# KIT-ISAS/lili-om

Measured on AMD Instinct MI355X. Metric: scan-to-map iterations/s (200k-pt scan vs 5M-pt map), higher is better.
Workload: dtype f64; 1 GPU; configs[2]: synthetic 64-ring 200000-pt scan vs 5000000-pt local map (variant A, seed 0x11110), ROT back-end matcher (surf), 1 outer GN iteration per step, a new registration from the perturbed pose every 10 steps, the 200k queries of the scan block-sharded over the ranks; queries_per_rank=200000, map_points=5000000, parallelism=single GPU, collectives=none, device_preheat_steps=2000

## Files before the change

lili_om_amd/csrc/lili_api.hip:

```cpp
#include "lili_launch.h"

#include <cmath>
#include <cstddef>
#include <cstdio>
#include <cstdlib>
#include <cstring>
#include <string>
#include <vector>

constexpr size_t kPinBytes = 64 * 1024;
namespace lili {
constexpr int kGatherMax = 12;
struct GatherTable { const unsigned char* src[kGatherMax]; unsigned off[kGatherMax], bytes[kGatherMax]; int n; };
__global__ __launch_bounds__(256) void k_readback_gather(GatherTable t, unsigned char* __restrict__ dst) {
    for (int k = 0; k < t.n; k++) {
        const unsigned char* s = t.src[k];
        unsigned char* d = dst + t.off[k];
        const unsigned nb = t.bytes[k];
        if (((reinterpret_cast<uintptr_t>(s) | reinterpret_cast<uintptr_t>(d) | nb) & 3u) == 0) {
            for (unsigned i = threadIdx.x; i < nb / 4; i += 256) reinterpret_cast<unsigned*>(d)[i] = reinterpret_cast<const unsigned*>(s)[i];
        } else for (unsigned i = threadIdx.x; i < nb; i += 256) d[i] = s[i];
    }
}
}
// ... 162 lines not shown
    if (!ctx) return LILI_E_ARG;
    HIPCHK(hipStreamSynchronize(ctx->stream));
    return LILI_OK;
}

int lili_set_debug(lili_ctx* ctx, int keep_neighbors) {
    if (!ctx) return LILI_E_ARG;
    ctx->keep_nn = keep_neighbors != 0;
    return LILI_OK;
}

int lili_set_option(lili_ctx* ctx, const char* name, int value) {
    if (!ctx || !name) return LILI_E_ARG;
    if (std::strcmp(name, "grid_reach") == 0) { if (value != 1 && value != 2) return ctx->fail(LILI_E_ARG, "grid_reach must be 1 or 2"); ctx->grid_reach = value; return LILI_OK; }
    if (std::strcmp(name, "cell_pct") == 0) { if (value < 50 || value > 100) return ctx->fail(LILI_E_ARG, "cell_pct must be in 50..100"); ctx->cell_pct = value; return LILI_OK; }
    if (std::strcmp(name, "fuse_tail") == 0) { ctx->fuse_tail = value != 0; return LILI_OK; }
    if (std::strcmp(name, "merge_kinds") == 0) { ctx->merge_kinds = value != 0; return LILI_OK; }
    if (std::strcmp(name, "fuse_lin") == 0) { ctx->fuse_lin = value != 0; return LILI_OK; }
    if (std::strcmp(name, "sort_fused_max_tiles") == 0) { ctx->sort_fused_max_tiles = std::max(0, value); return LILI_OK; }
    if (std::strcmp(name, "sort_fused_scan") == 0) { ctx->sort_fused_scan = value != 0; return LILI_OK; }
    if (std::strcmp(name, "persistent_iterate") == 0) { ctx->persistent_iterate = value != 0; return LILI_OK; }
    if (std::strcmp(name, "count_barrier") == 0) { ctx->count_barrier = value != 0; return LILI_OK; }
    if (std::strcmp(name, "assoc_lpq") == 0) {
        if (value != 0 && value != 1 && value != 2 && value != 4 && value != 8 && value != 16) return ctx->fail(LILI_E_ARG, "assoc_lpq must be 0 (auto), 1, 2, 4, 8 or 16");
        ctx->assoc_lpq = value; return LILI_OK;
    }
    if (std::strcmp(name, "fuse_lin_block") == 0) { if (value != 0 && value != kAssocBlock && value != kBlock) return ctx->fail(LILI_E_ARG, "fuse_lin_block must be 0 (auto), 64 or 256"); ctx->fuse_lin_block = value; return LILI_OK; }
    if (std::strcmp(name, "fine_grid") == 0) { ctx->fine_grid = value != 0; return LILI_OK; }
    if (std::strcmp(name, "sort_ride_hist") == 0) { ctx->sort_ride_hist = value != 0; return LILI_OK; }
    if (std::strcmp(name, "frame_guess_counts") == 0) { ctx->frame_guess_counts = value != 0; return LILI_OK; }
    if (std::strcmp(name, "frame_extract_stream") == 0) { ctx->frame_extract_stream = value != 0; return LILI_OK; }
    if (std::strcmp(name, "rot_fold") == 0) { ctx->rot_fold = value != 0; return LILI_OK; }
    if (std::strcmp(name, "rot_segment_wait") == 0) { ctx->rot_segment_wait = value != 0; return LILI_OK; }
    if (std::strcmp(name, "super_rows") == 0) { ctx->super_rows = value != 0; return LILI_OK; }
    if (std::strcmp(name, "fine_occupancy") == 0) { if (value < 2) return ctx->fail(LILI_E_ARG, "fine_occupancy must be >= 2"); ctx->fine_occupancy = value; return LILI_OK; }
    if (std::strcmp(name, "scan_lookback") == 0) { ctx->scan_lookback = value != 0; return LILI_OK; }
    if (std::strcmp(name, "map_narrow_counts") == 0) { ctx->map_narrow_counts = value != 0; for (auto& b : ctx->spec_box) b.wide_counts = false; return LILI_OK; }
    if (std::strcmp(name, "map_guess_box") == 0) { ctx->map_guess_box = value != 0; for (auto& b : ctx->spec_box) { const bool w = b.wide_counts; b = SpecBox{}; b.wide_counts = w; } return LILI_OK; }
    if (std::strcmp(name, "localmap_super_rows") == 0) { ctx->localmap_super_rows = value != 0; return LILI_OK; }
    if (std::strcmp(name, "localmap_incremental") == 0) { ctx->localmap_incremental = value != 0; return LILI_OK; }
    if (std::strcmp(name, "sort_digit_bits") == 0) { if (value != 4 && value != 8) return ctx->fail(LILI_E_ARG, "sort_digit_bits must be 4 or 8"); ctx->sort_digit_bits = value; return LILI_OK; }
    if (std::strcmp(name, "rot_atan") == 0) { if (value != 1 && value != 2) return ctx->fail(LILI_E_ARG, "rot_atan must be 1 or 2"); ctx->rot_atan = value; return LILI_OK; }
    if (std::strcmp(name, "p2p_fusion") == 0) { ctx->no_p2p_fusion = value == 0; return LILI_OK; }
    if (std::strcmp(name, "readback_gather") == 0) { ctx->readback_gather = value != 0; return LILI_OK; }
    if (std::strcmp(name, "voxel_guess_bits") == 0) { ctx->voxel_guess_bits = value != 0; return LILI_OK; }
    if (std::strcmp(name, "voxel_small") == 0) { ctx->voxel_small = value != 0; return LILI_OK; }
#ifdef LILI_OVERLAP_GN
    if (std::strcmp(name, "overlap_gn") == 0) { ctx->overlap_gn = value != 0; return LILI_OK; }
#endif
    if (std::strcmp(name, "archive_max_mb") == 0) { if (value < 0) return ctx->fail(LILI_E_ARG, "archive_max_mb must be >= 0 (0: unlimited)"); ctx->archive_max_mb = value; return LILI_OK; }
    if (std::strcmp(name, "archive_slab_mb") == 0) { if (value < 1 || value > 65536) return ctx->fail(LILI_E_ARG, "archive_slab_mb must be in 1..65536"); ctx->archive_slab_mb = value; return LILI_OK; }
    if (std::strcmp(name, "global_map_batch_points") == 0) {
        if (value < 1024 || value > (1 << 27)) return ctx->fail(LILI_E_ARG, "global_map_batch_points must be in 1024..2^27");
        ctx->global_map_batch_points = value; return LILI_OK;
    }
    if (std::strcmp(name, "max_cells") == 0) { if (value < 1) return ctx->fail(LILI_E_ARG, "max_cells must be positive"); ctx->max_cells = value; return LILI_OK; }
    return ctx->fail(LILI_E_ARG, std::string("unknown option ") + name);
}

}
```

lili_om_amd/csrc/lili_ctx.h:

```cpp
#pragma once
#include "../../include/lili_hip.h"
#include "lili_kernels.h"

#include <algorithm>
#include <cmath>
#include <cstdint>
#include <cstdlib>
#include <cstring>
#include <functional>
#include <string>
#include <utility>
#include <vector>

using namespace lili;

namespace lili_detail {

struct DevBuf {
    void* p = nullptr;
    size_t cap = 0;
    hipError_t ensure(size_t bytes) {
        if (bytes + 256 <= cap) return hipSuccess;
        if (p) { hipError_t e = hipFree(p); p = nullptr; cap = 0; if (e != hipSuccess) return e; }
        size_t want = bytes + bytes / 8 + 256;
// ... 112 lines not shown
    unsigned long long readback_gen = 0;
    struct PinItem { void* dst; size_t off, bytes; };
    std::vector<PinItem> h_pin_items;
    struct LazyItem { const void* src; size_t off, bytes; };
    std::vector<LazyItem> h_pin_lazy;
    unsigned char* h_pin_dev = nullptr;
    bool readback_gather = true;
    double* h_records = nullptr;
    double* h_records_dev = nullptr;
    int max_cells = 1 << 27;
    int grid_reach = 2;
    bool fuse_tail = false;
    bool no_p2p_fusion = false;
    bool merge_kinds = true;
    int cell_pct = 65;
    bool fine_grid = true;
    int fine_occupancy = 12;
    double focus[3] = {0, 0, 0}, focus_radius = 0;
    int fuse_lin_block = 0;
    int assoc_lpq = 0;
    bool count_barrier = false;

    bool persistent_off_now = false;
    bool persistent_iterate = false;
    bool frontend_commit_pending = false;
    int32_t frontend_map_raw = 0;
    bool voxel_guess_bits = true;
    bool hook_box_words_zero = false;
    std::function<int()> pre_sync_hook;
    bool voxel_small = true;
    bool overlap_gn = false;
    unsigned long long gn_seq = 0;
    bool fuse_lin = true;
    bool super_rows = true;
    bool scan_lookback = true;
    bool localmap_super_rows = false;
    bool localmap_incremental = true;
    int sort_fused_max_tiles = 256;
    bool sort_fused_scan = true;
    static constexpr int kExtractSide = 2;
    hipEvent_t extract_fork_ev = nullptr;
    bool frame_extract_stream = false, extract_side_next = false, extract_join_pending = false;
    bool rot_fold = true, rot_segment_wait = true;
    int frame_guess_misses = 0;
    bool frame_guess_counts = true;
    bool sort_ride_hist = true;
    int sort_digit_bits = 8;
    int rot_atan = 2;
    int n_simd = 0;
    void* ext_rot = nullptr;
    void (*ext_rot_free)(void*) = nullptr;
    void* ext_livox = nullptr;
    void (*ext_livox_free)(void*) = nullptr;
    void* ext_voxel = nullptr;
    void (*ext_voxel_free)(void*) = nullptr;
    void* ext_loop = nullptr;
    void (*ext_loop_free)(void*) = nullptr;
    void* ext_archive = nullptr;
    void (*ext_archive_free)(void*) = nullptr;
    int archive_max_mb = 0;
    int archive_slab_mb = 64;
    int global_map_batch_points = 1 << 21;

    int fail(int code, const std::string& m) { err = m; return code; }
    SlotState* state(int slot) { return states.as<SlotState>() + slot; }
    double* gram_of(int slot) { return gram.as<double>() + (size_t)slot * LILI_GRAM_DOUBLES; }
// ... 46 lines not shown
```

lili_om_amd/csrc/lili_kernels.h:

```cpp
#pragma once
#include <hip/hip_runtime.h>
#include <stdint.h>
#include "../../include/lili_hip.h"
#include "lili_p2p_dev.h"

namespace lili {

struct GridView {
    const float4* pts;
    const float* aux;
    const int* cell_start;
    const int* cell_start9;
    int bx0, by0, bz0, bnx, bny, bnz;
    double ox, oy, oz;
    double inv_cell;
    double cell;
    int nx, ny, nz;
    int n_points;
    int reach;
};

struct SrcCloud {
    const unsigned char* p;
    int stride, aux_off;
    int f4;
};

struct SlotState {
    double pose[7];
    int n_res[2];
    int gn_status;
    int iters;
    double last_delta[6];
    long long tprof[16];
    unsigned int reserved_;
    unsigned long long cnt_word;
    unsigned long long epoch;
    unsigned long long wait_failed;
};
constexpr int kPubReplicas = 64;
constexpr int kPubStride = 16;

struct FuseTail {
    int mode;
    const double* part_surf; int nb_surf;
    const double* part_edge; int nb_edge;
    double* out;
    SlotState* state;
    int debug;
    const SlotState* pose_src;
};

// ... 96 lines not shown
```

lili_om_amd/csrc/lili_match.hip:

```cpp
#include "lili_launch.h"

#include <cmath>
#include <cstddef>
#include <cstdio>
#include <cstdlib>
#include <cstring>
#include <string>
#include <type_traits>
#include <vector>

static MatchParams to_device_params(const lili_s2m_params* p) {
    MatchParams m{};
    m.variant = p->variant; m.loss = p->loss; m.loss_a = p->loss_a; m.lidar_const = p->lidar_const;
    m.kd_max_radius = p->kd_max_radius; m.edge_gate = p->edge_gate; m.surf_dist_thres = p->surf_dist_thres;
    m.reflect_thres = p->reflect_thres; m.surf_weight_min = p->surf_weight_min; m.edge_dist_max = p->edge_dist_max;
    for (int i = 0; i < 4; i++) m.q_lb[i] = p->q_lb[i];
    {
        const double w = p->q_lb[0], qx = p->q_lb[1], qy = p->q_lb[2], qz = p->q_lb[3];
        const double n2 = w * w + qx * qx + qy * qy + qz * qz;
        if (n2 > 0) { m.q_lb_inv[0] = w / n2; m.q_lb_inv[1] = -qx / n2; m.q_lb_inv[2] = -qy / n2; m.q_lb_inv[3] = -qz / n2; }
        else m.q_lb_inv[0] = m.q_lb_inv[1] = m.q_lb_inv[2] = m.q_lb_inv[3] = 0.0;
        const double gi = 1.0 / n2;
        if (n2 > 0) { m.q_lb_inv_jet[0] = w * gi; m.q_lb_inv_jet[1] = (-qx) * gi; m.q_lb_inv_jet[2] = (-qy) * gi; m.q_lb_inv_jet[3] = (-qz) * gi; }
        else m.q_lb_inv_jet[0] = m.q_lb_inv_jet[1] = m.q_lb_inv_jet[2] = m.q_lb_inv_jet[3] = 0.0;
// ... 28 lines not shown
    for (int i = 0; i < 4; i++) pa.q[i] = q[i];
    return pa;
}
static int derives_assoc(const lili_s2m_params* params) { return params->variant == LILI_VARIANT_FRONTEND ? 0 : 1; }
static PoseArg pose_of_slot(lili_ctx* ctx, int slot, const lili_s2m_params* assoc_params = nullptr, int pose_slot = -1) {
    PoseArg pa{};
    pa.state = ctx->state(pose_slot >= 0 ? pose_slot : slot);
    pa.derive_assoc = assoc_params ? derives_assoc(assoc_params) : 0;
    return pa;
}

static bool gate_fits(const MapIndex& m, int kind, const MatchParams& P) {
    const double gate = kind == LILI_KIND_SURF ? P.kd_max_radius : P.edge_gate;
    return std::sqrt(gate) * 1.0099 <= m.cell * (double)m.view.reach;
}
static bool livox_aux_ok(const MapIndex& m, const KindSlot& ks, int kind, const MatchParams& P) {
    return kind != LILI_KIND_SURF || P.variant != LILI_VARIANT_LIVOX || (m.has_aux && ks.has_aux);
}
static bool coop_eligible(lili_ctx* ctx, int slot, int kind_mask, const MatchParams& P, int64_t* n_all) {
    for (int kind = 0; kind < 2; kind++) if (kind_mask & (1 << kind)) {
        const KindSlot& ks = ctx->slots[slot].k[kind];
        const MapIndex& m = ctx->map[kind];
        if (!ks.has_queries || !m.valid || ks.n_q == 0 || m.n < 5 || m.has_fine) return false;
        if (!gate_fits(m, kind, P) || !livox_aux_ok(m, ks, kind, P)) return false;
        *n_all += ks.n_q;
    }
    return true;
}

static int assoc_args_of(lili_ctx* ctx, int slot, int kind, const GridView& view, int nb, int launches, AssocArgs& a) {
    KindSlot& ks = ctx->slots[slot].k[kind];
    const size_t n = (size_t)ks.n_q;
    a = AssocArgs{};
    a.queries = ks.q.as<float4>(); a.n_q = (int)n; a.g = view;
    a.rec0 = ks.rec0.as<float4>(); a.rec1 = ks.rec1.p; a.valid = ks.valid.as<unsigned char>();
    if (ctx->keep_nn) {
        HIPCHK(ks.dbg_idx.ensure(n * 5 * sizeof(int)));
        HIPCHK(ks.dbg_d2.ensure(n * 5 * sizeof(float)));
        a.dbg_idx = ks.dbg_idx.as<int>(); a.dbg_d2 = ks.dbg_d2.as<float>();
    }
    HIPCHK(ks.block_counts.ensure((size_t)nb * sizeof(int)));
    a.block_counts = ks.block_counts.as<int>(); a.nb = nb;
    ks.n_assoc_blocks = nb; ks.has_records = true; ks.launches += launches;
    return LILI_OK;
}
static int coop_args_of(lili_ctx* ctx, int slot, int kind_mask, int L, int launches, AssocArgs A[2]) {
    for (int kind = 0; kind < 2; kind++) {
        A[kind] = AssocArgs{};
        if (kind_mask & (1 << kind)) TRY(assoc_args_of(ctx, slot, kind, ctx->map[kind].view, nblocks(ctx->slots[slot].k[kind].n_q, 256 / L), launches, A[kind]));
    }
    return LILI_OK;
}

template <typename F> static bool with_lanes(int L, F&& f) {
    switch (L) {
        case 2: f(std::integral_constant<int, 2>{}); return true;
        case 4: f(std::integral_constant<int, 4>{}); return true;
        case 8: f(std::integral_constant<int, 8>{}); return true;
        case 16: f(std::integral_constant<int, 16>{}); return true;
        default: return false;
    }
}

constexpr size_t kHRecordDoubles = (size_t)LILI_MAX_SLOTS * LILI_GRAM_DOUBLES + 2 * LILI_MAX_SLOTS;
constexpr size_t kHWindowCountsOff = (size_t)LILI_MAX_SLOTS * LILI_GRAM_DOUBLES * sizeof(double), kHSlotCountsOff = kHWindowCountsOff + 2 * LILI_MAX_SLOTS * sizeof(int);
static int ensure_h_records(lili_ctx* ctx) {
    if (ctx->h_records) return LILI_OK;
// ... 1243 lines not shown
```

lili_om_amd/csrc/lili_s2m.hip:

```cpp
#include <type_traits>
#include "lili_kernels.h"
#include "lili_device_math.h"
#include "lili_device_cloud.h"
#include "lili_s2m_dev.h"

namespace lili {

__global__ __launch_bounds__(256) void k_cloud_to_f4(const unsigned char* __restrict__ raw, int n, int stride, int aux_off, float4* __restrict__ out, unsigned* __restrict__ mm) {
    float mn[3] = {INFINITY, INFINITY, INFINITY}, mx[3] = {-INFINITY, -INFINITY, -INFINITY};
    for (int i = blockIdx.x * blockDim.x + threadIdx.x; i < n; i += gridDim.x * blockDim.x) {
        const float4 v = load_row_f4(raw + (size_t)i * stride, aux_off);
        out[i] = v;
        if (mm && isfinite(v.x) && isfinite(v.y) && isfinite(v.z)) {
            mn[0] = fminf(mn[0], v.x); mn[1] = fminf(mn[1], v.y); mn[2] = fminf(mn[2], v.z);
            mx[0] = fmaxf(mx[0], v.x); mx[1] = fmaxf(mx[1], v.y); mx[2] = fmaxf(mx[2], v.z);
        }
    }
    if (!mm) return;
#pragma unroll
    for (int k = 0; k < 3; k++)
        for (int o = 32; o > 0; o >>= 1) { mn[k] = fminf(mn[k], __shfl_xor(mn[k], o)); mx[k] = fmaxf(mx[k], __shfl_xor(mx[k], o)); }
    __shared__ float smn[4][3], smx[4][3];
    if ((threadIdx.x & 63) == 0) {
#pragma unroll
// ... 546 lines not shown
        state->n_res[0] = t0; state->n_res[1] = t1;
        if (out) { out[0] = t0; out[1] = t1; }
    }
}



template <int BS, class TAB>
__device__ __forceinline__ void assoc_surf_body(
        const float4* __restrict__ queries, int n_q, const GridView& g, const PoseArg& pa, const MatchParams& P,
        float4* __restrict__ rec_nd, double* __restrict__ rec_score, unsigned char* __restrict__ valid,
        int* __restrict__ dbg_idx, float* __restrict__ dbg_d2, int* __restrict__ block_counts, int bid, TAB& tab, LaneRec* rec_out = nullptr) {
#ifdef LILI_PHASE_PROBE
    const long long t_begin = (P.debug & 4096) ? (long long)__builtin_amdgcn_s_memrealtime() : 0ll;
#endif
    const int i0 = bid * BS;
    const bool live = i0 + (int)threadIdx.x < n_q;
    const int i = live ? i0 + (int)threadIdx.x : 0;
    float4 ql = queries[i];
    dq Q2; d3 T2;
    load_assoc_pose(pa, P, Q2, T2);
    d3 pmd = qrot(Q2, d3{(double)ql.x, (double)ql.y, (double)ql.z}) + T2;
    float px = (float)pmd.x, py = (float)pmd.y, pz = (float)pmd.z;
    Top5 nn; nn.aux = 0; nn.have = false;
#ifdef LILI_PHASE_PROBE
    PhaseProbe probe;
#pragma unroll
    for (int k = 0; k < 8; k++) probe.t[k] = 0;
    PhaseProbe* const pp = &probe;
#else
    PhaseProbe* const pp = nullptr;
#endif
    PHASE_STAMP(pp, 1, px);
    if (live) knn5_grid(g, tab, px, py, pz, gate_bound(P.kd_max_radius), nn, P.debug, pp);
    bool ok = false;
    if (live) {
        store_debug_nn(g, nn, i, dbg_idx, dbg_d2);
        float4 rn; double score;
        ok = surf_fit(g, P, nn, ql, px, py, pz, rn, score);
        PHASE_STAMP(pp, 6, rn.w);
        rec_nd[i] = rn;
        rec_score[i] = score;
        valid[i] = ok ? 1 : 0;
        if (rec_out) { rec_out->ql = ql; rec_out->r0 = rn; rec_out->score = score; }
    }
    if (rec_out) rec_out->ok = ok;
    store_block_count<BS>(ok, block_counts, bid);
#ifdef LILI_PHASE_PROBE
    if ((P.debug & 4096) && dbg_d2 && threadIdx.x == 0) {
        for (int k = 1; k <= 6; k++) dbg_d2[(size_t)i0 * 5 + k] = probe.t[k] ? (float)(probe.t[k] - t_begin) : -1.0f;
    }
    if ((P.debug & 4096) && dbg_idx && threadIdx.x == 0) {
        long long* o = (long long*)(dbg_idx + (size_t)i0 * 5);
        unsigned hw, xcc;
        asm volatile("s_getreg_b32 %0, hwreg(HW_REG_HW_ID)" : "=s"(hw));
        asm volatile("s_getreg_b32 %0, hwreg(HW_REG_XCC_ID)" : "=s"(xcc));
        o[0] = t_begin; o[1] = (long long)__builtin_amdgcn_s_memrealtime();
        dbg_idx[(size_t)i0 * 5 + 4] = (int)((hw & 0xffffu) | (xcc << 16));
    }
    if ((P.debug & 4096) && dbg_idx && live && threadIdx.x != 0) dbg_idx[(size_t)i * 5] = nn.aux;
#endif
}
template <int BS>
__global__ __launch_bounds__(BS) void k_associate_surf(
        const float4* __restrict__ queries, int n_q, GridView g, PoseArg pa, MatchParams P,
        float4* __restrict__ rec_nd, double* __restrict__ rec_score, unsigned char* __restrict__ valid,
        int* __restrict__ dbg_idx, float* __restrict__ dbg_d2, int* __restrict__ block_counts) {
    __shared__ RowTabT<BS> tab;
    assoc_surf_body<BS>(queries, n_q, g, pa, P, rec_nd, rec_score, valid, dbg_idx, dbg_d2, block_counts, (int)blockIdx.x, tab);
}

template <int BS, class TAB>
__device__ __forceinline__ void assoc_edge_body(
        const float4* __restrict__ queries, int n_q, const GridView& g, const PoseArg& pa, const MatchParams& P,
        float4* __restrict__ rec_a, float4* __restrict__ rec_b, unsigned char* __restrict__ valid,
        int* __restrict__ dbg_idx, float* __restrict__ dbg_d2, int* __restrict__ block_counts, int bid, TAB& tab, LaneRec* rec_out = nullptr) {
    const int i0 = bid * BS;
    const bool live = i0 + (int)threadIdx.x < n_q;
    const int i = live ? i0 + (int)threadIdx.x : 0;
    float4 ql = queries[i];
    dq Q2; d3 T2;
    load_assoc_pose(pa, P, Q2, T2);
    d3 pmd = qrot(Q2, d3{(double)ql.x, (double)ql.y, (double)ql.z}) + T2;
    float px = (float)pmd.x, py = (float)pmd.y, pz = (float)pmd.z;
    Top5 nn; nn.have = false;
    if (live) knn5_grid(g, tab, px, py, pz, gate_bound(P.edge_gate), nn);
    bool ok = false;
    if (live) {
        store_debug_nn(g, nn, i, dbg_idx, dbg_d2);
        float4 ra, rb;
        ok = edge_fit(g, P, nn, px, py, pz, ra, rb);
        rec_a[i] = ra; rec_b[i] = rb; valid[i] = ok ? 1 : 0;
        if (rec_out) { rec_out->ql = ql; rec_out->r0 = ra; rec_out->r1 = rb; }
    }
    if (rec_out) rec_out->ok = ok;
    store_block_count<BS>(ok, block_counts, bid);
}
template <int BS>
__global__ __launch_bounds__(BS) void k_associate_edge(
        const float4* __restrict__ queries, int n_q, GridView g, PoseArg pa, MatchParams P,
        float4* __restrict__ rec_a, float4* __restrict__ rec_b, unsigned char* __restrict__ valid,
        int* __restrict__ dbg_idx, float* __restrict__ dbg_d2, int* __restrict__ block_counts) {
    __shared__ RowTabT<BS> tab;
    assoc_edge_body<BS>(queries, n_q, g, pa, P, rec_a, rec_b, valid, dbg_idx, dbg_d2, block_counts, (int)blockIdx.x, tab);
}

__global__ __launch_bounds__(kAssocBlock) void k_associate_both(AssocArgs S, AssocArgs E, PoseArg pa, MatchParams P) {
    __shared__ RowTabT<kAssocBlock> tab;
    const int b = (int)blockIdx.x;
    if (b < E.nb) assoc_edge_body<kAssocBlock>(E.queries, E.n_q, E.g, pa, P, E.rec0, reinterpret_cast<float4*>(E.rec1), E.valid, E.dbg_idx, E.dbg_d2, E.block_counts, b, tab);
    else assoc_surf_body<kAssocBlock>(S.queries, S.n_q, S.g, pa, P, S.rec0, reinterpret_cast<double*>(S.rec1), S.valid, S.dbg_idx, S.dbg_d2, S.block_counts, b - E.nb, tab);
}
template __global__ void k_associate_surf<kAssocBlock>(const float4*, int, GridView, PoseArg, MatchParams, float4*, double*, unsigned char*, int*, float*, int*);
template __global__ void k_associate_edge<kAssocBlock>(const float4*, int, GridView, PoseArg, MatchParams, float4*, float4*, unsigned char*, int*, float*, int*);


template <bool XCHG>
__device__ __forceinline__ void reduce_partials_block(const double* part_surf, int nb_surf, const double* part_edge, int nb_edge,
                                                      double* __restrict__ out, SlotState* __restrict__ state, int do_gn, unsigned long long key, const P2PView& xv,
// ... 463 lines not shown
```

lili_om_amd/csrc/lili_s2m_dev.h:

```cpp
#pragma once
#include <type_traits>
#include "lili_kernels.h"
#include "lili_device_math.h"

namespace lili {

__device__ __forceinline__ int cell_coord(float v, double o, double inv_cell) {
    return (int)floor(((double)v - o) * inv_cell);
}
__device__ __forceinline__ int cell_of(float4 p, const GridView& g) {
    if (!(isfinite(p.x) && isfinite(p.y) && isfinite(p.z))) return 0;
    int cx = min(max(cell_coord(p.x, g.ox, g.inv_cell), 0), g.nx - 1);
    int cy = min(max(cell_coord(p.y, g.oy, g.inv_cell), 0), g.ny - 1);
    int cz = min(max(cell_coord(p.z, g.oz, g.inv_cell), 0), g.nz - 1);
    return (cz * g.ny + cy) * g.nx + cx;
}

__device__ __forceinline__ size_t srow_index(const GridView& g, int x, int y, int z) {
    return ((size_t)(z - g.bz0) * (size_t)g.bny + (size_t)(y - g.by0)) * (size_t)g.bnx + (size_t)(x - g.bx0);
}

struct Top5 {
    float d[5];
    int j[5];
    int aux;
    float4 p[5];
    bool have;
};
__device__ __forceinline__ float dist2(float4 p, float qx, float qy, float qz) {
    float r = 0.f;
    float dx = qx - p.x; r += dx * dx;
    float dy = qy - p.y; r += dy * dy;
    float dz = qz - p.z; r += dz * dz;
    return r;
}
struct Sel5 {
    unsigned long long k[5];
    int j[5];
    __device__ __forceinline__ void init(float bound = 3.0e38f) {
        bound = fminf(bound, 3.0e38f);
#pragma unroll
        for (int s = 0; s < 5; s++) { k[s] = ((unsigned long long)__float_as_uint(bound) << 32) | 0x7fffffffull; j[s] = -1; }
    }
    __device__ __forceinline__ void insert(float d, float4 p, int jpos) {
        const unsigned long long key = ((unsigned long long)__float_as_uint(d) << 32) | (unsigned)__float_as_int(p.w);
        const bool c0 = key < k[0], c1 = key < k[1], c2 = key < k[2], c3 = key < k[3], c4 = key < k[4];
        k[4] = c3 ? k[3] : (c4 ? key : k[4]);  j[4] = c3 ? j[3] : (c4 ? jpos : j[4]);
        k[3] = c2 ? k[2] : (c3 ? key : k[3]);  j[3] = c2 ? j[2] : (c3 ? jpos : j[3]);
        k[2] = c1 ? k[1] : (c2 ? key : k[2]);  j[2] = c1 ? j[1] : (c2 ? jpos : j[2]);
        k[1] = c0 ? k[0] : (c1 ? key : k[1]);  j[1] = c0 ? j[0] : (c1 ? jpos : j[1]);
        k[0] = c0 ? key : k[0];                j[0] = c0 ? jpos : j[0];
    }
    __device__ __forceinline__ float worst() const { return __uint_as_float((unsigned)(k[4] >> 32)); }
    __device__ __forceinline__ bool final_tie() const { return false; }
    __device__ __forceinline__ unsigned worst_bits() const { return (unsigned)(k[4] >> 32); }
    __device__ __forceinline__ void to_top5(Top5& t) const {
#pragma unroll
        for (int s = 0; s < 5; s++) { t.d[s] = __uint_as_float((unsigned)(k[s] >> 32)); t.j[s] = j[s]; }
        t.have = false;
    }
};

__device__ __forceinline__ unsigned umed3(unsigned a, unsigned b, unsigned c) {
    unsigned r;
    asm("v_med3_u32 %0, %1, %2, %3" : "=v"(r) : "v"(a), "v"(b), "v"(c));
    return r;
}
struct Sel5K {
    unsigned k[6];
    int tc;
    int* T;
    int ts;
    unsigned bb;
    float bnd;
    __device__ __forceinline__ void init(float bound) {
        bnd = fminf(bound, 3.0e38f);
        bb = __float_as_uint(bnd) >> 6;
#pragma unroll
        for (int s = 0; s < 6; s++) k[s] = ((bb + 1u + (unsigned)s) << 6) | 63u;
        tc = 0; T = nullptr; ts = 0;
    }
    __device__ __forceinline__ void attach(int* col, int stride) { T = col; ts = stride; T[15 * stride] = -4; }
    __device__ __forceinline__ float worst() const { return __uint_as_float(k[4] | 63u); }
    __device__ __forceinline__ unsigned worst_bits() const { return k[4] | 63u; }
    __device__ __forceinline__ void to_top5(Top5& t) const {
#pragma unroll
        for (int s = 0; s < 5; s++) { t.d[s] = bnd; t.j[s] = -1; }
        t.have = false;
    }
    __device__ __forceinline__ void push(unsigned key) {
        const unsigned m5 = umed3(k[4], k[5], key), m4 = umed3(k[3], k[4], key), m3 = umed3(k[2], k[3], key);
        const unsigned m2 = umed3(k[1], k[2], key), m1 = umed3(k[0], k[1], key);
        k[0] = min(k[0], key); k[1] = m1; k[2] = m2; k[3] = m3; k[4] = m4; k[5] = m5;
    }
    __device__ __forceinline__ int where(unsigned key) const { const unsigned c = key & 63u; return T[(int)(c >> 2) * ts] + (int)(c & 3u); }
    __device__ __forceinline__ void repoint() {
        int jr[6];
#pragma unroll
        for (int s = 0; s < 6; s++) jr[s] = where(k[s]);
#pragma unroll
        for (int s = 0; s < 6; s++) { T[(8 + s) * ts] = jr[s]; k[s] = (k[s] & ~63u) | (unsigned)(32 + 4 * s); }
    }
    __device__ __forceinline__ void chunk(float4 p0, float4 p1, float4 p2, float4 p3, int j, int end, float qx, float qy, float qz) {
        if (tc >= 8 && (tc & 7) == 0) repoint();
        T[(tc & 7) * ts] = j;
        const unsigned code = (unsigned)(tc & 7) << 2;
        tc++;
        const unsigned u0 = __float_as_uint(dist2(p0, qx, qy, qz));
        const unsigned u1 = j + 1 < end ? __float_as_uint(dist2(p1, qx, qy, qz)) : 0x7f800000u;
        const unsigned u2 = j + 2 < end ? __float_as_uint(dist2(p2, qx, qy, qz)) : 0x7f800000u;
        const unsigned u3 = j + 3 < end ? __float_as_uint(dist2(p3, qx, qy, qz)) : 0x7f800000u;
        push((u0 & ~63u) | code); push((u1 & ~63u) | (code + 1u)); push((u2 & ~63u) | (code + 2u)); push((u3 & ~63u) | (code + 3u));
    }
    __device__ __forceinline__ bool finish(const GridView& g, float qx, float qy, float qz, Top5& t) const {
        const bool redo = ((k[5] ^ k[4]) < 64u) || ((k[4] >> 6) == bb);
        unsigned long long e[5];
        int jr[5];
        float4 pp[5];
#pragma unroll
        for (int s = 0; s < 5; s++) {
            jr[s] = where(k[s]);
            const bool real = jr[s] >= 0;
            const float4 p = g.pts[real ? jr[s] : 0];
            pp[s] = p;
            const unsigned du = real ? __float_as_uint(dist2(p, qx, qy, qz)) : __float_as_uint(bnd);
            const unsigned lo = real ? (unsigned)__float_as_int(p.w) : 0x7fffffffu;
            e[s] = ((unsigned long long)du << 32) | lo;
        }
        const bool unsorted = !(e[0] <= e[1] && e[1] <= e[2] && e[2] <= e[3] && e[3] <= e[4]);
        if (__any(unsorted)) {
#define LILI_CE(a, b) { const bool sw = e[b] < e[a]; const unsigned long long ea = e[a], eb = e[b]; const int ja = jr[a], jb = jr[b]; \
                        const float4 pa_ = pp[a], pb_ = pp[b]; \
                        e[a] = sw ? eb : ea; e[b] = sw ? ea : eb; jr[a] = sw ? jb : ja; jr[b] = sw ? ja : jb; \
                        pp[a].x = sw ? pb_.x : pa_.x; pp[a].y = sw ? pb_.y : pa_.y; pp[a].z = sw ? pb_.z : pa_.z; pp[a].w = sw ? pb_.w : pa_.w; \
                        pp[b].x = sw ? pa_.x : pb_.x; pp[b].y = sw ? pa_.y : pb_.y; pp[b].z = sw ? pa_.z : pb_.z; pp[b].w = sw ? pa_.w : pb_.w; }
            LILI_CE(0, 1) LILI_CE(3, 4) LILI_CE(2, 4) LILI_CE(2, 3) LILI_CE(0, 3) LILI_CE(0, 2) LILI_CE(1, 4) LILI_CE(1, 3) LILI_CE(1, 2)
#undef LILI_CE
        }
#pragma unroll
        for (int s = 0; s < 5; s++) { t.d[s] = __uint_as_float((unsigned)(e[s] >> 32)); t.j[s] = jr[s]; t.p[s] = pp[s]; }
        t.aux = tc;
        t.have = !redo;
        return redo;
    }
};
// ... 95 lines not shown
    if (u2 <= sel.worst_bits()) sel.insert(__uint_as_float(u2), p2, min(j + 2, last));
    if (u3 <= sel.worst_bits()) sel.insert(__uint_as_float(u3), p3, min(j + 3, last));
}
template <class SEL>
__device__ __forceinline__ void scan_run(const GridView& g, SEL& sel, int beg, int end, float qx, float qy, float qz) {
    const int last = end - 1;
    for (int j = beg; j < end; j += 4) {
        float4 p0 = load_pt(g, j), p1 = load_pt(g, min(j + 1, last)), p2 = load_pt(g, min(j + 2, last)), p3 = load_pt(g, min(j + 3, last));
        process_chunk(sel, p0, p1, p2, p3, j, end, qx, qy, qz);
    }
}

template <int BS>
struct RowTabT {
    int b[9][BS];
    int e[9][BS];
    float lb[9][BS];
    int cj[16][BS];
};

struct PhaseProbe { long long t[8]; };
#ifdef LILI_PHASE_PROBE
#define PHASE_STAMP(pp, k, dep) do { if (pp) { long long t_; asm volatile("s_memrealtime %0\n\ts_waitcnt lgkmcnt(0)" : "=s"(t_) : "v"(dep) : "memory"); (pp)->t[k] = t_; } } while (0)
#else
#define PHASE_STAMP(pp, k, dep) do {} while (0)
#endif
__device__ __forceinline__ float gate_bound(double gate) {
    float gf = (float)gate;
    if ((double)gf < gate) gf = __uint_as_float(__float_as_uint(gf) + 1u);
    return gf;
}
__device__ constexpr int kShellDy[16] = {0, 0, -2, 2, -1, 1, -1, 1, -2, -2, 2, 2, -2, -2, 2, 2};
__device__ constexpr int kShellDz[16] = {-2, 2, 0, 0, -2, -2, 2, 2, -1, 1, -1, 1, -2, 2, -2, 2};
template <class SEL, class TAB>
__device__ __forceinline__ bool knn5_grid_sel(const GridView& g, TAB& tab, float qx, float qy, float qz, float bound, Top5& best, PhaseProbe* pp = nullptr) {
    SEL sel; sel.init(bound);
    sel.to_top5(best);
    if (!(isfinite(qx) && isfinite(qy) && isfinite(qz))) return false;
    if constexpr (std::is_same<SEL, Sel5K>::value) sel.attach(&tab.cj[0][threadIdx.x], (int)(sizeof(tab.cj[0]) / sizeof(int)));
    const int R = g.reach;
    int cx = cell_coord(qx, g.ox, g.inv_cell), cy = cell_coord(qy, g.oy, g.inv_cell), cz = cell_coord(qz, g.oz, g.inv_cell);
    if (cx < -R || cx > g.nx - 1 + R || cy < -R || cy > g.ny - 1 + R || cz < -R || cz > g.nz - 1 + R) return false;
    const bool inner9 = g.cell_start9 && cy >= g.by0 && cy < g.by0 + g.bny && cz >= g.bz0 && cz < g.bz0 + g.bnz &&
                        max(cx - 1, 0) >= g.bx0 && min(cx + 1, g.nx - 1) < g.bx0 + g.bnx;
    if (inner9) {
        const int x0 = max(cx - 1, 0), x1 = min(cx + 1, g.nx - 1);
        if (x0 <= x1) {
            const int* row = g.cell_start9 + srow_index(g, g.bx0, cy, cz) - g.bx0;
            int cj = row[x0];
            const int ce = row[x1 + 1];
            PHASE_STAMP(pp, 2, ce);
            auto fetch = [&](float4& p0, float4& p1, float4& p2, float4& p3, int& pj) {
                pj = cj;
                const float4* q = (const float4*)((const char*)g.pts + ((unsigned)cj << 4));
                p0 = q[0]; p1 = q[1]; p2 = q[2]; p3 = q[3];
                cj += 4;
            };
            float4 a0, a1, a2, a3, b0, b1, b2, b3;
            int aj = 0, bj = 0;
            fetch(a0, a1, a2, a3, aj);
            for (;;) {
                if (!(aj < ce)) break;
                fetch(b0, b1, b2, b3, bj);
                process_chunk(sel, a0, a1, a2, a3, aj, ce, qx, qy, qz);
                if (!(bj < ce)) break;
                fetch(a0, a1, a2, a3, aj);
                process_chunk(sel, b0, b1, b2, b3, bj, ce, qx, qy, qz);
            }
        }
    } else {
        const int x0 = max(cx - 1, 0), x1 = min(cx + 1, g.nx - 1);
        if (x0 <= x1) {
            int rb[9], re[9];
#pragma unroll
            for (int n = 0; n < 9; n++) {
                const int w = row_order(n);
                const int y = cy + w / 3 - 1, z = cz + w % 3 - 1;
                const bool in = z >= 0 && z < g.nz && y >= 0 && y < g.ny;
// ... 18 lines not shown
                while (cj >= ce && n < cnt) {
                    const int b = tab.b[n][tid], e = tab.e[n][tid];
                    const float lb = tab.lb[n][tid];
                    n++;
                    if (!(lb > wv)) { cj = b; ce = e; }
                }
                pj = cj; pe = ce;
                if (cj < ce) {
                    const int last = ce - 1;
                    p0 = load_pt(g, cj); p1 = load_pt(g, min(cj + 1, last)); p2 = load_pt(g, min(cj + 2, last)); p3 = load_pt(g, min(cj + 3, last));
                    cj += 4;
                }
            };
            float4 a0, a1, a2, a3, b0, b1, b2, b3;
            int aj = 0, ae = 0, bj = 0, be = 0;
            fetch(sel.worst(), a0, a1, a2, a3, aj, ae);
            for (;;) {
                if (!(aj < ae)) break;
                fetch(sel.worst(), b0, b1, b2, b3, bj, be);
                process_chunk(sel, a0, a1, a2, a3, aj, ae, qx, qy, qz);
                if (!(bj < be)) break;
                fetch(sel.worst(), a0, a1, a2, a3, aj, ae);
                process_chunk(sel, b0, b1, b2, b3, bj, be, qx, qy, qz);
            }
        }
    }
    PHASE_STAMP(pp, 3, sel.worst());
    if (R == 2) {
        const double c = g.cell;
        const double fxm = (double)qx - (g.ox + (double)cx * c), fxp = (g.ox + (double)(cx + 1) * c) - (double)qx;
        const double fym = (double)qy - (g.oy + (double)cy * c), fyp = (g.oy + (double)(cy + 1) * c) - (double)qy;
        const double fzm = (double)qz - (g.oz + (double)cz * c), fzp = (g.oz + (double)(cz + 1) * c) - (double)qz;
        const double margin = c + fmax(fmin(fmin(fmin(fxm, fxp), fmin(fym, fyp)), fmin(fzm, fzp)), 0.0);
        if (!(sel.worst() < (float)(0.999 * margin * margin))) {
            const bool side9 = inner9 && (cx - 2 < 0 || cx - 2 >= g.bx0) && (cx + 2 >= g.nx || cx + 2 < g.bx0 + g.bnx);
            if (side9) {
                const int* row = g.cell_start9 + srow_index(g, g.bx0, cy, cz) - g.bx0;
                const int xl = cx - 2, xr = cx + 2;
                if (xl >= 0 && xl < g.nx) { const double gx = fmax(fxm + c, 0.0); if (!((float)(0.999 * gx * gx) > sel.worst())) scan_run(g, sel, row[xl], row[xl + 1], qx, qy, qz); }
                if (xr >= 0 && xr < g.nx) { const double gx = fmax(fxp + c, 0.0); if (!((float)(0.999 * gx * gx) > sel.worst())) scan_run(g, sel, row[xr], row[xr + 1], qx, qy, qz); }
            }
            const bool few = __popcll(__ballot(1)) <= 2;
            if (side9 && few) {
                const double g1m = fmax(fxm, 0.0), g1p = fmax(fxp, 0.0), g2m = fmax(fxm + c, 0.0), g2p = fmax(fxp + c, 0.0);
                const int tid = threadIdx.x;
#pragma unroll
                for (int batch = 0; batch < 2; batch++) {
                    const float wv = sel.worst();
                    int rb[8], re[8]; float rl[8];
#pragma unroll
                    for (int i = 0; i < 8; i++) {
                        const int dy = kShellDy[batch * 8 + i], dz = kShellDz[batch * 8 + i];
                        const int y = cy + dy, z = cz + dz;
                        const double gy = dy == 0 ? 0.0 : fmax(dy < 0 ? fym + (double)(-dy - 1) * c : fyp + (double)(dy - 1) * c, 0.0);
                        const double gz = dz == 0 ? 0.0 : fmax(dz < 0 ? fzm + (double)(-dz - 1) * c : fzp + (double)(dz - 1) * c, 0.0);
                        const double lbr = 0.999 * (gy * gy + gz * gz);
                        const int dl = (float)(lbr + 0.999 * g2m * g2m) > wv ? ((float)(lbr + 0.999 * g1m * g1m) > wv ? 0 : 1) : 2;
                        const int dr = (float)(lbr + 0.999 * g2p * g2p) > wv ? ((float)(lbr + 0.999 * g1p * g1p) > wv ? 0 : 1) : 2;
                        const int x0 = max(cx - dl, 0), x1 = min(cx + dr, g.nx - 1);
                        const bool keep = y >= 0 && y < g.ny && z >= 0 && z < g.nz && !((float)lbr > wv) && x0 <= x1;
                        const int* cs = g.cell_start + (size_t)(keep ? z * g.ny + y : 0) * g.nx;
                        const int b = cs[keep ? x0 : 0], e = cs[keep ? x1 + 1 : 0];
                        rb[i] = b; re[i] = keep ? e : b; rl[i] = (float)lbr;
                    }
#pragma unroll
                    for (int i = 0; i < 8; i++) { tab.b[i][tid] = rb[i]; tab.e[i][tid] = re[i]; tab.lb[i][tid] = rl[i]; }
                    for (int i = 0; i < 8; i++) {
                        const int b = tab.b[i][tid], e = tab.e[i][tid];
                        if (b < e && !(tab.lb[i][tid] > sel.worst())) scan_run(g, sel, b, e, qx, qy, qz);
                    }
                }
            } else
            for (int dz = -2; dz <= 2; dz++) {
                const int z = cz + dz;
                if (z < 0 || z >= g.nz) continue;
                const double gz = dz == 0 ? 0.0 : fmax(dz < 0 ? fzm + (double)(-dz - 1) * c : fzp + (double)(dz - 1) * c, 0.0);
                for (int dy = -2; dy <= 2; dy++) {
                    const int y = cy + dy;
                    if (y < 0 || y >= g.ny) continue;
                    const double gy = dy == 0 ? 0.0 : fmax(dy < 0 ? fym + (double)(-dy - 1) * c : fyp + (double)(dy - 1) * c, 0.0);
                    const double lbr = 0.999 * (gy * gy + gz * gz);
                    if ((float)lbr > sel.worst()) continue;
                    const int* cs = g.cell_start + (size_t)(z * g.ny + y) * g.nx;
                    if (dy == -2 || dy == 2 || dz == -2 || dz == 2) {
                        const float wv = sel.worst();
                        const double g1m = fmax(fxm, 0.0), g1p = fmax(fxp, 0.0), g2m = fmax(fxm + c, 0.0), g2p = fmax(fxp + c, 0.0);
                        const int dl = (float)(lbr + 0.999 * g2m * g2m) > wv ? ((float)(lbr + 0.999 * g1m * g1m) > wv ? 0 : 1) : 2;
                        const int dr = (float)(lbr + 0.999 * g2p * g2p) > wv ? ((float)(lbr + 0.999 * g1p * g1p) > wv ? 0 : 1) : 2;
                        const int x0 = max(cx - dl, 0), x1 = min(cx + dr, g.nx - 1);
                        if (x0 <= x1) scan_run(g, sel, cs[x0], cs[x1 + 1], qx, qy, qz);
                    } else if (!side9) {
                        const int xl = cx - 2, xr = cx + 2;
                        if (xl >= 0 && xl < g.nx) { double gx = fmax(fxm + c, 0.0); if (!((float)(lbr + 0.999 * gx * gx) > sel.worst())) scan_run(g, sel, cs[xl], cs[xl + 1], qx, qy, qz); }
                        if (xr >= 0 && xr < g.nx) { double gx = fmax(fxp + c, 0.0); if (!((float)(lbr + 0.999 * gx * gx) > sel.worst())) scan_run(g, sel, cs[xr], cs[xr + 1], qx, qy, qz); }
                    }
                }
            }
        }
    }
    PHASE_STAMP(pp, 4, sel.worst());
    if constexpr (std::is_same<SEL, Sel5K>::value) return sel.finish(g, qx, qy, qz, best);
    else { sel.to_top5(best); return sel.final_tie(); }
}
template <class TAB>
__device__ __forceinline__ void knn5_grid(const GridView& g, TAB& tab, float qx, float qy, float qz, float bound, Top5& best, int dbg = 0, PhaseProbe* pp = nullptr) {
    if (dbg & 32768) { knn5_grid_sel<Sel5>(g, tab, qx, qy, qz, bound, best); return; }
    const bool redo = knn5_grid_sel<Sel5K>(g, tab, qx, qy, qz, bound, best, pp);
    PHASE_STAMP(pp, 5, best.d[4]);
    if (redo) knn5_grid_sel<Sel5>(g, tab, qx, qy, qz, bound, best);
}

template <int BS>
__device__ __forceinline__ void store_block_count(bool ok, int* __restrict__ block_counts, int bid) {
    __shared__ int wave_cnt[BS / 64];
    unsigned long long bal = __ballot(ok);
    if ((threadIdx.x & 63) == 0) wave_cnt[threadIdx.x >> 6] = __popcll(bal);
    __syncthreads();
    if (threadIdx.x == 0) {
        int s = 0;
#pragma unroll
        for (int w = 0; w < BS / 64; w++) s += wave_cnt[w];
        block_counts[bid] = s;
    }
}
__device__ __forceinline__ int sum_block_counts_begin(const int* __restrict__ block_counts, int nb) {
    int s = 0;
    const int bd = blockDim.x;
    for (int b0 = threadIdx.x; b0 < nb; b0 += 4 * bd) {
        const int b1 = b0 + bd, b2 = b0 + 2 * bd, b3 = b0 + 3 * bd;
        const int v0 = block_counts[b0], v1 = b1 < nb ? block_counts[b1] : 0, v2 = b2 < nb ? block_counts[b2] : 0, v3 = b3 < nb ? block_counts[b3] : 0;
        s += (v0 + v1) + (v2 + v3);
    }
    for (int o = 32; o > 0; o >>= 1) s += __shfl_xor(s, o);
    return s;
}
__device__ __forceinline__ int sum_block_counts_end(int wave_sum) {
    __shared__ int part[16];
    __shared__ int total;
    if ((threadIdx.x & 63) == 0) part[threadIdx.x >> 6] = wave_sum;
    __syncthreads();
// ... 422 lines not shown
```

Before: 32360 iterations/s.

## Cooperatively scan kNN shell rows across a wave when few lanes need them

Adds a wave-cooperative path for the outer-shell kNN walk. When only a few lanes in a wavefront need the 16-row shell search, the lanes are regrouped so that 16 of them scan one query's shell rows in parallel. Candidates are exchanged through the LDS row table and merged into the owning lane's selector. This targets divergence, where one or two lanes walk 16 rows serially while the rest of the wave idles. In exchange it adds LDS traffic, wave barriers, and extra shuffles and double-precision work per round, and it makes every lane, including inactive ones, enter the kNN routine.

```diff
diff --git a/lili_om_amd/csrc/lili_api.hip b/lili_om_amd/csrc/lili_api.hip
--- a/lili_om_amd/csrc/lili_api.hip
+++ b/lili_om_amd/csrc/lili_api.hip
@@ -218,6 +218,7 @@
     if (std::strcmp(name, "frame_extract_stream") == 0) { ctx->frame_extract_stream = value != 0; return LILI_OK; }
     if (std::strcmp(name, "rot_fold") == 0) { ctx->rot_fold = value != 0; return LILI_OK; }
     if (std::strcmp(name, "rot_segment_wait") == 0) { ctx->rot_segment_wait = value != 0; return LILI_OK; }
+    if (std::strcmp(name, "shell_coop") == 0) { if (value < 0 || value > 64) return ctx->fail(LILI_E_ARG, "shell_coop must be in 0..64"); ctx->shell_coop = value; return LILI_OK; }
     if (std::strcmp(name, "super_rows") == 0) { ctx->super_rows = value != 0; return LILI_OK; }
     if (std::strcmp(name, "fine_occupancy") == 0) { if (value < 2) return ctx->fail(LILI_E_ARG, "fine_occupancy must be >= 2"); ctx->fine_occupancy = value; return LILI_OK; }
     if (std::strcmp(name, "scan_lookback") == 0) { ctx->scan_lookback = value != 0; return LILI_OK; }
diff --git a/lili_om_amd/csrc/lili_ctx.h b/lili_om_amd/csrc/lili_ctx.h
--- a/lili_om_amd/csrc/lili_ctx.h
+++ b/lili_om_amd/csrc/lili_ctx.h
@@ -168,6 +168,7 @@
     bool overlap_gn = false;
     unsigned long long gn_seq = 0;
     bool fuse_lin = true;
+    int shell_coop = 1;
     bool super_rows = true;
     bool scan_lookback = true;
     bool localmap_super_rows = false;
diff --git a/lili_om_amd/csrc/lili_kernels.h b/lili_om_amd/csrc/lili_kernels.h
--- a/lili_om_amd/csrc/lili_kernels.h
+++ b/lili_om_amd/csrc/lili_kernels.h
@@ -18,6 +18,7 @@
     int nx, ny, nz;
     int n_points;
     int reach;
+    int shell_coop;
 };
 
 struct SrcCloud {
diff --git a/lili_om_amd/csrc/lili_match.hip b/lili_om_amd/csrc/lili_match.hip
--- a/lili_om_amd/csrc/lili_match.hip
+++ b/lili_om_amd/csrc/lili_match.hip
@@ -84,7 +84,7 @@
     KindSlot& ks = ctx->slots[slot].k[kind];
     const size_t n = (size_t)ks.n_q;
     a = AssocArgs{};
-    a.queries = ks.q.as<float4>(); a.n_q = (int)n; a.g = view;
+    a.queries = ks.q.as<float4>(); a.n_q = (int)n; a.g = view; a.g.shell_coop = ctx->shell_coop;
     a.rec0 = ks.rec0.as<float4>(); a.rec1 = ks.rec1.p; a.valid = ks.valid.as<unsigned char>();
     if (ctx->keep_nn) {
         HIPCHK(ks.dbg_idx.ensure(n * 5 * sizeof(int)));
diff --git a/lili_om_amd/csrc/lili_s2m.hip b/lili_om_amd/csrc/lili_s2m.hip
--- a/lili_om_amd/csrc/lili_s2m.hip
+++ b/lili_om_amd/csrc/lili_s2m.hip
@@ -602,7 +602,7 @@
     PhaseProbe* const pp = nullptr;
 #endif
     PHASE_STAMP(pp, 1, px);
-    if (live) knn5_grid(g, tab, px, py, pz, gate_bound(P.kd_max_radius), nn, P.debug, pp);
+    knn5_grid_wave(g, tab, live, px, py, pz, gate_bound(P.kd_max_radius), nn, P.debug, pp);
     bool ok = false;
     if (live) {
         store_debug_nn(g, nn, i, dbg_idx, dbg_d2);
@@ -654,7 +654,7 @@
     d3 pmd = qrot(Q2, d3{(double)ql.x, (double)ql.y, (double)ql.z}) + T2;
     float px = (float)pmd.x, py = (float)pmd.y, pz = (float)pmd.z;
     Top5 nn; nn.have = false;
-    if (live) knn5_grid(g, tab, px, py, pz, gate_bound(P.edge_gate), nn);
+    knn5_grid_wave(g, tab, live, px, py, pz, gate_bound(P.edge_gate), nn);
     bool ok = false;
     if (live) {
         store_debug_nn(g, nn, i, dbg_idx, dbg_d2);
diff --git a/lili_om_amd/csrc/lili_s2m_dev.h b/lili_om_amd/csrc/lili_s2m_dev.h
--- a/lili_om_amd/csrc/lili_s2m_dev.h
+++ b/lili_om_amd/csrc/lili_s2m_dev.h
@@ -42,8 +42,7 @@
 #pragma unroll
         for (int s = 0; s < 5; s++) { k[s] = ((unsigned long long)__float_as_uint(bound) << 32) | 0x7fffffffull; j[s] = -1; }
     }
-    __device__ __forceinline__ void insert(float d, float4 p, int jpos) {
-        const unsigned long long key = ((unsigned long long)__float_as_uint(d) << 32) | (unsigned)__float_as_int(p.w);
+    __device__ __forceinline__ void insert_key(unsigned long long key, int jpos) {
         const bool c0 = key < k[0], c1 = key < k[1], c2 = key < k[2], c3 = key < k[3], c4 = key < k[4];
         k[4] = c3 ? k[3] : (c4 ? key : k[4]);  j[4] = c3 ? j[3] : (c4 ? jpos : j[4]);
         k[3] = c2 ? k[2] : (c3 ? key : k[3]);  j[3] = c2 ? j[2] : (c3 ? jpos : j[3]);
@@ -51,6 +50,7 @@
         k[1] = c0 ? k[0] : (c1 ? key : k[1]);  j[1] = c0 ? j[0] : (c1 ? jpos : j[1]);
         k[0] = c0 ? key : k[0];                j[0] = c0 ? jpos : j[0];
     }
+    __device__ __forceinline__ void insert(float d, float4 p, int jpos) { insert_key(((unsigned long long)__float_as_uint(d) << 32) | (unsigned)__float_as_int(p.w), jpos); }
     __device__ __forceinline__ float worst() const { return __uint_as_float((unsigned)(k[4] >> 32)); }
     __device__ __forceinline__ bool final_tie() const { return false; }
     __device__ __forceinline__ unsigned worst_bits() const { return (unsigned)(k[4] >> 32); }
@@ -111,6 +111,13 @@
         const unsigned u2 = j + 2 < end ? __float_as_uint(dist2(p2, qx, qy, qz)) : 0x7f800000u;
         const unsigned u3 = j + 3 < end ? __float_as_uint(dist2(p3, qx, qy, qz)) : 0x7f800000u;
         push((u0 & ~63u) | code); push((u1 & ~63u) | (code + 1u)); push((u2 & ~63u) | (code + 2u)); push((u3 & ~63u) | (code + 3u));
+    }
+    __device__ __forceinline__ void push_one(unsigned u, int j) {
+        if (tc >= 8 && (tc & 7) == 0) repoint();
+        T[(tc & 7) * ts] = j;
+        const unsigned code = (unsigned)(tc & 7) << 2;
+        tc++;
+        push((u & ~63u) | code);
     }
     __device__ __forceinline__ bool finish(const GridView& g, float qx, float qy, float qz, Top5& t) const {
         const bool redo = ((k[5] ^ k[4]) < 64u) || ((k[4] >> 6) == bb);
@@ -272,18 +279,92 @@
 }
 __device__ constexpr int kShellDy[16] = {0, 0, -2, 2, -1, 1, -1, 1, -2, -2, 2, 2, -2, -2, 2, 2};
 __device__ constexpr int kShellDz[16] = {-2, 2, 0, 0, -2, -2, 2, 2, -1, 1, -1, 1, -2, 2, -2, 2};
-template <class SEL, class TAB>
-__device__ __forceinline__ bool knn5_grid_sel(const GridView& g, TAB& tab, float qx, float qy, float qz, float bound, Top5& best, PhaseProbe* pp = nullptr) {
+__device__ __forceinline__ void wave_lds_sync() { __builtin_amdgcn_fence(__ATOMIC_ACQ_REL, "wavefront"); __builtin_amdgcn_wave_barrier(); }
+constexpr unsigned long long pack_shell_rows(const int (&a)[16]) { unsigned long long v = 0; for (int i = 0; i < 16; i++) v |= (unsigned long long)(a[i] + 2) << (4 * i); return v; }
+template <class TAB>
+__device__ __forceinline__ void shell_coop_pass(const GridView& g, TAB& tab, Sel5K& sel, unsigned long long bal, bool need, float qx, float qy, float qz, int cx, int cy, int cz) {
+    constexpr int kShDy[16] = {0, 0, -2, 2, -1, 1, -1, 1, -2, -2, 2, 2, -2, -2, 2, 2}, kShDz[16] = {-2, 2, 0, 0, -2, -2, 2, 2, -1, 1, -1, 1, -2, 2, -2, 2};
+    constexpr unsigned long long kDy = pack_shell_rows(kShDy), kDz = pack_shell_rows(kShDz);
+    constexpr int BS = (int)(sizeof(tab.b[0]) / sizeof(int));
+    const int n = __popcll(bal);
+    const int lane = (int)(threadIdx.x & 63u), wb = (int)(threadIdx.x & ~63u), grp = lane >> 4, sub = lane & 15;
+    int* const area = &tab.b[0][0] + wb;
+    static_assert(sizeof(tab.b) == 9 * BS * sizeof(int) && sizeof(tab.e) == sizeof(tab.b), "row table layout");
+    auto cellp = [&](int idx) -> int* { return area + (idx >> 6) * BS + (idx & 63); };
+    const int rank = __popcll(bal & ((1ull << lane) - 1ull));
+    if (need) *cellp(rank) = lane;
+    wave_lds_sync();
+    const int dy = (int)((kDy >> (4 * sub)) & 15ull) - 2, dz = (int)((kDz >> (4 * sub)) & 15ull) - 2;
+    const double c = g.cell;
+    float oqx = 0.f, oqy = 0.f, oqz = 0.f;
+    auto prepare = [&](int r0, float& ox_, float& oy_, float& oz_, int& b, int& e) {
+        const int qi = r0 + grp;
+        const int o = *cellp(min(qi, n - 1));
+        ox_ = __shfl(qx, o); oy_ = __shfl(qy, o); oz_ = __shfl(qz, o);
+        const float wv = __shfl(sel.worst(), o);
+        const int ocx = __shfl(cx, o), ocy = __shfl(cy, o), ocz = __shfl(cz, o);
+        const double fxm = (double)ox_ - (g.ox + (double)ocx * c), fxp = (g.ox + (double)(ocx + 1) * c) - (double)ox_;
+        const double fym = (double)oy_ - (g.oy + (double)ocy * c), fyp = (g.oy + (double)(ocy + 1) * c) - (double)oy_;
+        const double fzm = (double)oz_ - (g.oz + (double)ocz * c), fzp = (g.oz + (double)(ocz + 1) * c) - (double)oz_;
+        const double g1m = fmax(fxm, 0.0), g1p = fmax(fxp, 0.0), g2m = fmax(fxm + c, 0.0), g2p = fmax(fxp + c, 0.0);
+        const int y = ocy + dy, z = ocz + dz;
+        const double gy = dy == 0 ? 0.0 : fmax(dy < 0 ? fym + (double)(-dy - 1) * c : fyp + (double)(dy - 1) * c, 0.0);
+        const double gz = dz == 0 ? 0.0 : fmax(dz < 0 ? fzm + (double)(-dz - 1) * c : fzp + (double)(dz - 1) * c, 0.0);
+        const double lbr = 0.999 * (gy * gy + gz * gz);
+        const int dl = (float)(lbr + 0.999 * g2m * g2m) > wv ? ((float)(lbr + 0.999 * g1m * g1m) > wv ? 0 : 1) : 2;
+        const int dr = (float)(lbr + 0.999 * g2p * g2p) > wv ? ((float)(lbr + 0.999 * g1p * g1p) > wv ? 0 : 1) : 2;
+        const int x0 = max(ocx - dl, 0), x1 = min(ocx + dr, g.nx - 1);
+        const bool keep = qi < n && y >= 0 && y < g.ny && z >= 0 && z < g.nz && !((float)lbr > wv) && x0 <= x1;
+        const int* cs = g.cell_start + (size_t)(keep ? z * g.ny + y : 0) * g.nx;
+        b = cs[keep ? x0 : 0];
+        const int e1 = cs[keep ? x1 + 1 : 0];
+        e = keep ? e1 : b;
+        return wv;
+    };
+    int b = 0, e = 0;
+    float wv = prepare(0, oqx, oqy, oqz, b, e);
+    for (int r0 = 0; r0 < n; r0 += 4) {
+        float nqx = 0.f, nqy = 0.f, nqz = 0.f, nwv = 0.f;
+        int nb = 0, ne = 0;
+        if (r0 + 4 < n) nwv = prepare(r0 + 4, nqx, nqy, nqz, nb, ne);
+        Sel5 hs; hs.init(wv);
+        scan_run(g, hs, b, e, oqx, oqy, oqz);
+        int cnt = 0;
+#pragma unroll
+        for (int s = 0; s < 5; s++) {
+            const bool has = hs.j[s] >= 0;
+            const unsigned m = (unsigned)(__ballot(has) >> (16 * grp)) & 0xffffu;
+            if (has) {
+                const int at = 64 + grp * 160 + 2 * (cnt + __popc(m & ((1u << sub) - 1u)));
+                *cellp(at) = (int)(unsigned)(hs.k[s] >> 32); *cellp(at + 1) = hs.j[s];
+            }
+            cnt += __popc(m);
+        }
+        wave_lds_sync();
+        const int mine = (rank - r0) & 3;
+        const int mcnt = __shfl(cnt, mine << 4);
+        if (need && rank >= r0 && rank < r0 + 4) {
+            for (int t = 0; t < mcnt; t++) { const int at = 64 + mine * 160 + 2 * t; sel.push_one((unsigned)*cellp(at), *cellp(at + 1)); }
+        }
+        wave_lds_sync();
+        oqx = nqx; oqy = nqy; oqz = nqz; wv = nwv; b = nb; e = ne;
+    }
+}
+template <class SEL, class TAB, bool WAVE = false>
+__device__ __forceinline__ bool knn5_grid_sel(const GridView& g, TAB& tab, float qx, float qy, float qz, float bound, Top5& best, PhaseProbe* pp = nullptr, bool live = true) {
     SEL sel; sel.init(bound);
     sel.to_top5(best);
-    if (!(isfinite(qx) && isfinite(qy) && isfinite(qz))) return false;
+    bool act = live && isfinite(qx) && isfinite(qy) && isfinite(qz);
+    if (!WAVE && !act) return false;
     if constexpr (std::is_same<SEL, Sel5K>::value) sel.attach(&tab.cj[0][threadIdx.x], (int)(sizeof(tab.cj[0]) / sizeof(int)));
     const int R = g.reach;
-    int cx = cell_coord(qx, g.ox, g.inv_cell), cy = cell_coord(qy, g.oy, g.inv_cell), cz = cell_coord(qz, g.oz, g.inv_cell);
-    if (cx < -R || cx > g.nx - 1 + R || cy < -R || cy > g.ny - 1 + R || cz < -R || cz > g.nz - 1 + R) return false;
+    int cx = act ? cell_coord(qx, g.ox, g.inv_cell) : 0, cy = act ? cell_coord(qy, g.oy, g.inv_cell) : 0, cz = act ? cell_coord(qz, g.oz, g.inv_cell) : 0;
+    if (cx < -R || cx > g.nx - 1 + R || cy < -R || cy > g.ny - 1 + R || cz < -R || cz > g.nz - 1 + R) act = false;
+    if (!WAVE && !act) return false;
     const bool inner9 = g.cell_start9 && cy >= g.by0 && cy < g.by0 + g.bny && cz >= g.bz0 && cz < g.bz0 + g.bnz &&
                         max(cx - 1, 0) >= g.bx0 && min(cx + 1, g.nx - 1) < g.bx0 + g.bnx;
-    if (inner9) {
+    if (!act) {
+    } else if (inner9) {
         const int x0 = max(cx - 1, 0), x1 = min(cx + 1, g.nx - 1);
         if (x0 <= x1) {
             const int* row = g.cell_start9 + srow_index(g, g.bx0, cy, cz) - g.bx0;
@@ -368,8 +449,23 @@
         const double fym = (double)qy - (g.oy + (double)cy * c), fyp = (g.oy + (double)(cy + 1) * c) - (double)qy;
         const double fzm = (double)qz - (g.oz + (double)cz * c), fzp = (g.oz + (double)(cz + 1) * c) - (double)qz;
         const double margin = c + fmax(fmin(fmin(fmin(fxm, fxp), fmin(fym, fyp)), fmin(fzm, fzp)), 0.0);
-        if (!(sel.worst() < (float)(0.999 * margin * margin))) {
-            const bool side9 = inner9 && (cx - 2 < 0 || cx - 2 >= g.bx0) && (cx + 2 >= g.nx || cx + 2 < g.bx0 + g.bnx);
+        const bool shell = act && !(sel.worst() < (float)(0.999 * margin * margin));
+        const bool side9 = inner9 && (cx - 2 < 0 || cx - 2 >= g.bx0) && (cx + 2 >= g.nx || cx + 2 < g.bx0 + g.bnx);
+        bool walk = shell;
+        if constexpr (WAVE && std::is_same<SEL, Sel5K>::value) {
+            const unsigned long long bal = __ballot(shell && side9);
+            if (g.shell_coop && bal && __popcll(bal) <= (g.shell_coop == 1 ? 16 : g.shell_coop)) {
+                if (shell && side9) {
+                    const int* row = g.cell_start9 + srow_index(g, g.bx0, cy, cz) - g.bx0;
+                    const int xl = cx - 2, xr = cx + 2;
+                    if (xl >= 0 && xl < g.nx) { const double gx = fmax(fxm + c, 0.0); if (!((float)(0.999 * gx * gx) > sel.worst())) scan_run(g, sel, row[xl], row[xl + 1], qx, qy, qz); }
+                    if (xr >= 0 && xr < g.nx) { const double gx = fmax(fxp + c, 0.0); if (!((float)(0.999 * gx * gx) > sel.worst())) scan_run(g, sel, row[xr], row[xr + 1], qx, qy, qz); }
+                }
+                shell_coop_pass(g, tab, sel, bal, shell && side9, qx, qy, qz, cx, cy, cz);
+                walk = shell && !side9;
+            }
+        }
+        if (walk) {
             if (side9) {
                 const int* row = g.cell_start9 + srow_index(g, g.bx0, cy, cz) - g.bx0;
                 const int xl = cx - 2, xr = cx + 2;
@@ -435,6 +531,7 @@
         }
     }
     PHASE_STAMP(pp, 4, sel.worst());
+    if (WAVE && !act) return false;
     if constexpr (std::is_same<SEL, Sel5K>::value) return sel.finish(g, qx, qy, qz, best);
     else { sel.to_top5(best); return sel.final_tie(); }
 }
@@ -442,6 +539,13 @@
 __device__ __forceinline__ void knn5_grid(const GridView& g, TAB& tab, float qx, float qy, float qz, float bound, Top5& best, int dbg = 0, PhaseProbe* pp = nullptr) {
     if (dbg & 32768) { knn5_grid_sel<Sel5>(g, tab, qx, qy, qz, bound, best); return; }
     const bool redo = knn5_grid_sel<Sel5K>(g, tab, qx, qy, qz, bound, best, pp);
+    PHASE_STAMP(pp, 5, best.d[4]);
+    if (redo) knn5_grid_sel<Sel5>(g, tab, qx, qy, qz, bound, best);
+}
+template <class TAB>
+__device__ __forceinline__ void knn5_grid_wave(const GridView& g, TAB& tab, bool live, float qx, float qy, float qz, float bound, Top5& best, int dbg = 0, PhaseProbe* pp = nullptr) {
+    if (dbg & 32768) { if (live) knn5_grid_sel<Sel5>(g, tab, qx, qy, qz, bound, best); return; }
+    const bool redo = knn5_grid_sel<Sel5K, TAB, true>(g, tab, qx, qy, qz, bound, best, pp, live);
     PHASE_STAMP(pp, 5, best.d[4]);
     if (redo) knn5_grid_sel<Sel5>(g, tab, qx, qy, qz, bound, best);
 }
```

Result: no change. 32480 iterations/s, median of 6 (+0.4%).
